# kokkos/kokkos-kernels

Hardware: AMD Instinct MI355X
Metric: SpMV GFLOP/s (CSR, 27-pt 3-D FE Laplacian, fp64) (higher is better)
Workload: dtype f64

## Files before the change

kokkos-kernels_amd/csrc/kk_spmv.hip:

```cpp
#include "kk_common.h"
#include "kk_scan.h"
#include <new>
#include <cstring>
#include <climits>

#include "kk_spmv_plan.h"

namespace kk {

template <class OffT, class AT, class YT, int LPR>
__global__ __launch_bounds__(kBlock) void spmv_vector_kernel(int64_t nrows, const OffT* __restrict__ row_map,
                                                             const int32_t* __restrict__ entries,
                                                             const AT* __restrict__ values, const YT* __restrict__ x,
                                                             YT* __restrict__ y, YT alpha, YT beta, int remap) {
  constexpr int RPB = kBlock / LPR;
  const int64_t wg  = remap ? xcd_remap(blockIdx.x, gridDim.x) : (int64_t)blockIdx.x;
  const int64_t row = wg * RPB + threadIdx.x / LPR;
  const int lane    = threadIdx.x % LPR;
  YT sum            = YT(0);
  if (row < nrows) {
    const OffT s = row_map[row], e = row_map[row + 1];
    for (OffT j = s + lane; j < e; j += LPR) sum += (YT)values[j] * x[entries[j]];
  }
  sum = group_sum(sum, LPR);
// ... 440 lines not shown
  const int mode = tinfo[b] & 3;
  if (mode == kTilePattern) { if (threadIdx.x == 0) tinfo[b] = mode | (int32_t)((unsigned)b << 2); return; }
  if (mode != kTileCodes && mode != kTileStaged) return;
  const int64_t d = idx[b];
  const kk_u32x4* src = reinterpret_cast<const kk_u32x4*>(full + b * TILE);
  kk_u32x4* dst       = reinterpret_cast<kk_u32x4*>(compact + d * TILE);
  for (int i = threadIdx.x; i < TILE / 8; i += kBlock) dst[i] = src[i];
  if (threadIdx.x == 0) tinfo[b] = mode | (int32_t)((unsigned)d << 2);
}

template <class AT, int STEPS, bool FULL, bool NT = false>
__device__ __forceinline__ void load_tile_values(const AT* __restrict__ values, int64_t ts, int64_t te, int t, AT (&v0)[STEPS],
                                                 AT (&v1)[STEPS]) {
  using AV = typename vec2<AT>::type;
  constexpr int SPAN = kBlock * 2;
  KK_UNROLL
  for (int k = 0; k < STEPS; ++k) {
    const int64_t idx = ts + (int64_t)k * SPAN + t * 2;
    if (FULL || idx + 1 < te) {
      const AV* vp = reinterpret_cast<const AV*>(values + idx);
      const AV vv  = NT ? KK_NT_LOAD(vp) : *vp;
      v0[k] = vv[0]; v1[k] = vv[1];
    } else if (idx < te) {
      v0[k] = values[idx]; v1[k] = AT(0);
    } else {
      v0[k] = v1[k] = AT(0);
    }
  }
}

template <int STEPS, bool NT = false>
__device__ __forceinline__ void load_tile_codes(const uint16_t* __restrict__ wtile, int t, unsigned (&w)[STEPS]) {
  constexpr int NPT = 2 * STEPS;
  const unsigned* cw = reinterpret_cast<const unsigned*>(wtile + t * NPT);
  if (STEPS % 4 == 0) {
    KK_UNROLL
    for (int k = 0; k < STEPS; k += 4) {
      const kk_u32x4* qp = reinterpret_cast<const kk_u32x4*>(cw + k);
      const kk_u32x4 q   = NT ? KK_NT_LOAD(qp) : *qp;
      w[k] = q[0]; w[k + 1] = q[1]; w[k + 2] = q[2]; w[k + 3] = q[3];
    }
  } else {
    KK_UNROLL
    for (int k = 0; k < STEPS; k += 2) {
      const kk_u32x2* qp = reinterpret_cast<const kk_u32x2*>(cw + k);
      const kk_u32x2 q   = NT ? KK_NT_LOAD(qp) : *qp;
      w[k] = q[0]; w[k + 1] = q[1];
    }
  }
}

#ifdef KK_EMU
#define KK_USE_AFTER_ISSUE(v)
#else
#define KK_USE_AFTER_ISSUE(v) asm volatile("" : "+v"(v))
#endif

template <class AT, int STEPS, bool FULL>
__device__ __forceinline__ void load_tile_win(const AT* __restrict__ values, const uint16_t* __restrict__ wtile,
                                              const int32_t* __restrict__ wmeta, int64_t b, int64_t ts, int64_t te, int t,
                                              AT (&v0)[STEPS], AT (&v1)[STEPS], int (&c0)[STEPS], int (&c1)[STEPS]) {
  constexpr int SPAN = kBlock * 2;
  unsigned w[STEPS];
  load_tile_codes<STEPS>(wtile, t, w);
  const int meta = wmeta[b * kWinMeta + (t & (kWinMeta - 1))];
  load_tile_values<AT, STEPS, FULL>(values, ts, te, t, v0, v1);
  KK_UNROLL
  for (int k = 0; k < STEPS; ++k) KK_USE_AFTER_ISSUE(w[k]);
  KK_UNROLL
  for (int k = 0; k < STEPS; ++k) {
    const int64_t idx = ts + (int64_t)k * SPAN + t * 2;
    const unsigned lo = w[k] & 0xffffu, hi = w[k] >> 16;
    const int b0 = __shfl(meta, (int)(lo >> kWinBits), 64), b1 = __shfl(meta, (int)(hi >> kWinBits), 64);
    c0[k] = b0 + (int)(lo & ((1u << kWinBits) - 1));
    c1[k] = b1 + (int)(hi & ((1u << kWinBits) - 1));
    if (!FULL) {
      if (idx >= te) c0[k] = c1[k] = -1;
      else if (idx + 1 >= te) c1[k] = c0[k];
    }
  }
}

template <class AT, int STEPS> struct WinTile { AT v0[STEPS], v1[STEPS]; unsigned w[STEPS]; int meta, prec0; };

template <class AT, int STEPS, bool FULL, bool NT, bool PAT>
__device__ __forceinline__ void win_issue(const AT* __restrict__ values, const uint16_t* __restrict__ wtile,
                                          const int32_t* __restrict__ wmeta, const int32_t* __restrict__ pmeta, int64_t b,
                                          int64_t ts, int64_t te, int t, WinTile<AT, STEPS>& W) {
  W.meta  = wmeta[b * kWinMeta + (t & 63)];
  W.prec0 = 0;
  if (PAT) W.prec0 = pmeta[b * kPatW + (t < kPatW ? t : kPatW - 1)];
  load_tile_values<AT, STEPS, FULL, NT>(values, ts, te, t, W.v0, W.v1);
  if (!PAT) load_tile_codes<STEPS, NT>(wtile, t, W.w);
}

template <class AT, class YT, int STEPS, bool PAT>
__device__ __forceinline__ void win_stage(WinTile<AT, STEPS>& W, const YT* __restrict__ x, int64_t ncols, YT* prod, int64_t b, int t,
                                          const int32_t* __restrict__ pmeta) {
  constexpr int SPAN = kBlock * 2, NPT = 2 * STEPS, TILE = kBlock * NPT;
  constexpr int CAPC = (TILE < kWinChunks * 64 ? TILE : kWinChunks * 64) / 64;
  constexpr int CPW  = (CAPC + kBlock / 64 - 1) / (kBlock / 64);
  constexpr int GRP  = STEPS < 4 ? STEPS : 4;
  const AT (&v0)[STEPS] = W.v0;
  const AT (&v1)[STEPS] = W.v1;
  const unsigned (&w)[STEPS] = W.w;
  const int lane = t & 63, wave = t >> 6;
  const int meta = W.meta;
  const int32_t* pm = PAT ? pmeta + b * kPatW : nullptr;
  const int nseg    = PAT ? pm[0] : 0;
  YT xv[CPW];
  bool used[CPW];
  KK_UNROLL
  for (int i = 0; i < CPW; ++i) {
    const int c   = wave + i * (kBlock / 64);
    const int col = c < CAPC ? __shfl(meta, 2 * kWinCount + c, 64) : -1;
    used[i]       = col >= 0;
    int64_t xi    = (int64_t)(used[i] ? col : 0) + lane;
    xi            = xi < ncols ? xi : ncols - 1;
    xv[i]         = x[xi];
  }
  KK_UNROLL
  for (int i = 0; i < CPW; ++i) {
    const int c = wave + i * (kBlock / 64);
    if (used[i]) prod[c * 64 + lane] = xv[i];
  }
  int* sseg = reinterpret_cast<int*>(prod + TILE) - kPatW;
  const short* stab = reinterpret_cast<const short*>(sseg + kPatTab);
  if (PAT && t < kPatW) sseg[t] = W.prec0;
  __syncthreads();
  YT x0[STEPS], x1[STEPS];
  if (PAT) {
    if (nseg == 1) {
      const int jadd = pm[kPatRec + 1];
      const unsigned L = (unsigned)pm[kPatRec + 2];
      const float rcp  = __int_as_float(pm[kPatRec + 3]);
      KK_UNROLL
      for (int k = 0; k < STEPS; ++k) {
        KK_UNROLL
        for (int h = 0; h < 2; ++h) {
          const unsigned j   = (unsigned)(k * SPAN + t * 2 + h + jadd);
          const unsigned row = (unsigned)(((float)j + 0.5f) * rcp);
          const int slot     = (int)stab[(int)(j - KK_UMUL24(row, L))] + (int)row;
          if (h == 0) x0[k] = prod[slot]; else x1[k] = prod[slot];
        }
      }
    } else if (nseg <= 4) {
      const int sb1 = pm[1], sb2 = pm[2], sb3 = pm[3];
      const int ja0 = pm[kPatRec + 1], ja1 = pm[kPatRec + 5], ja2 = pm[kPatRec + 9], ja3 = pm[kPatRec + 13];
      const int sl0 = pm[kPatRec + 2], sl1 = pm[kPatRec + 6], sl2 = pm[kPatRec + 10], sl3 = pm[kPatRec + 14];
      const int sm0 = pm[kPatRec + 3], sm1 = pm[kPatRec + 7], sm2 = pm[kPatRec + 11], sm3 = pm[kPatRec + 15];
      KK_UNROLL
      for (int k0 = 0; k0 < STEPS; k0 += GRP) {
        int ti[2 * GRP], rw[2 * GRP], sl[2 * GRP];
        KK_UNROLL
        for (int q = 0; q < 2 * GRP; ++q) {
          const int li  = (k0 + q / 2) * SPAN + t * 2 + (q & 1);
          const bool c1 = li >= sb1, c2 = li >= sb2, c3 = li >= sb3;
          const int ja  = c3 ? ja3 : c2 ? ja2 : c1 ? ja1 : ja0;
          const int sl_ = c3 ? sl3 : c2 ? sl2 : c1 ? sl1 : sl0;
          const int sm  = c3 ? sm3 : c2 ? sm2 : c1 ? sm1 : sm0;
          const int tb  = c3 ? 3 * kPatLen : c2 ? 2 * kPatLen : c1 ? kPatLen : 0;
          const unsigned j   = (unsigned)(li + ja);
          const unsigned row = (unsigned)(((float)j + 0.5f) * __int_as_float(sm));
          ti[q] = tb + (int)(j - KK_UMUL24(row, (unsigned)sl_));
          rw[q] = (int)row;
        }
        KK_UNROLL
        for (int q = 0; q < 2 * GRP; ++q) sl[q] = (int)stab[ti[q]] + rw[q];
        KK_UNROLL
        for (int q = 0; q < 2 * GRP; ++q) {
          if ((q & 1) == 0) x0[k0 + q / 2] = prod[sl[q]]; else x1[k0 + q / 2] = prod[sl[q]];
        }
      }
    } else {
      const int sb1 = pm[1], sb2 = pm[2], sb3 = pm[3], sb4 = pm[4], sb5 = pm[5], sb6 = pm[6], sb7 = pm[7];
      KK_UNROLL
// ... 79 lines not shown
      vb[k] = quad_pick<0xFA, AT>(v0[k], v1[k], odd);
    }
    KK_UNROLL
    for (int k = 0; k < STEPS; ++k) {
      const int li = k * SPAN + t * 2 - j;
      prod[li]     = (YT)va[k] * xa[k];
      prod[li + 4] = (YT)vb[k] * xb[k];
    }
    return;
  }
  YT x0[STEPS], x1[STEPS];
  KK_UNROLL
  for (int k = 0; k < STEPS; ++k) {
    x0[k] = (FULL || c0[k] >= 0) ? x[FULL ? c0[k] : (c0[k] >= 0 ? c0[k] : 0)] : YT(0);
    x1[k] = (FULL || c1[k] >= 0) ? x[FULL ? c1[k] : (c1[k] >= 0 ? c1[k] : 0)] : YT(0);
  }
  KK_UNROLL
  for (int k = 0; k < STEPS; ++k) {
    const int li = k * SPAN + t * 2;
    prod[li]     = (YT)v0[k] * x0[k];
    prod[li + 1] = (YT)v1[k] * x1[k];
  }
}

template <class YT> __device__ __forceinline__ YT strided_lds_sum(const YT* prod, int i0, int i1, int lane, int G) {
  YT s0 = YT(0), s1 = YT(0), s2 = YT(0), s3 = YT(0);
  int i = i0 + lane;
  const int G2 = 2 * G, G3 = 3 * G, G4 = 4 * G;
  for (; i + G3 < i1; i += G4) {
    const YT a = prod[i], b = prod[i + G], c = prod[i + G2], d = prod[i + G3];
    s0 += a; s1 += b; s2 += c; s3 += d;
  }
  for (; i < i1; i += G) s0 += prod[i];
  return (s0 + s1) + (s2 + s3);
}

template <class OffT, class AT, class YT, int NPT, int MODE>
__global__ __launch_bounds__(kBlock) void spmv_stream3_kernel(int64_t nnz, const OffT* __restrict__ row_map,
                                                              const int32_t* __restrict__ entries,
                                                              const AT* __restrict__ values, const YT* __restrict__ x,
                                                              YT* __restrict__ y, YT alpha, YT beta,
                                                              const int32_t* __restrict__ blk_info,
                                                              YT* __restrict__ carry_head, YT* __restrict__ carry_tail,
                                                              int remap, const int32_t* __restrict__ list,
                                                              const int32_t* __restrict__ tinfo,
                                                              const uint16_t* __restrict__ wcode,
                                                              const int32_t* __restrict__ wmeta, int64_t ncols,
                                                              const int32_t* __restrict__ pmeta KK_ABL_PARAM) {
  constexpr int TILE  = kBlock * NPT;
  constexpr int STEPS = NPT / 2;
  __shared__ YT prod[TILE];
  constexpr bool NT = false;
  const int t       = threadIdx.x;
  const int64_t pos = xcd_order(blockIdx.x, gridDim.x, remap);
  const int64_t b   = list ? (int64_t)list[pos] : pos;
  const int64_t s = b * TILE;
  const bool full = (s + TILE <= nnz);
  const int64_t e = full ? s + TILE : nnz;

  const int32_t info0 = blk_info[b], info1 = blk_info[b + 1];
  const uint16_t* wtile = nullptr;
  if (MODE == kTileCodes || MODE == kTileStaged) wtile = wcode + (int64_t)((unsigned)tinfo[b] >> 2) * TILE;

  AT v0[STEPS], v1[STEPS];
  int c0[STEPS], c1[STEPS];
  WinTile<AT, STEPS> W;
  if (MODE == kTilePattern) {
    win_issue<AT, STEPS, true, NT, true>(values, wtile, wmeta, pmeta, b, s, e, t, W);
  } else if (MODE == kTileStaged) {
    if (full) win_issue<AT, STEPS, true, NT, false>(values, wtile, wmeta, pmeta, b, s, e, t, W);
    else      win_issue<AT, STEPS, false, NT, false>(values, wtile, wmeta, pmeta, b, s, e, t, W);
  } else if (MODE == kTileCodes) {
    if (full) load_tile_win<AT, STEPS, true>(values, wtile, wmeta, b, s, e, t, v0, v1, c0, c1);
    else      load_tile_win<AT, STEPS, false>(values, wtile, wmeta, b, s, e, t, v0, v1, c0, c1);
  } else {
    if (full) load_tile<AT, STEPS, NT, true>(values, entries, s, e, t, v0, v1, c0, c1);
    else      load_tile<AT, STEPS, NT, false>(values, entries, s, e, t, v0, v1, c0, c1);
  }

  const int64_t ra    = info0 & 0x7fffffff;
  const int64_t rb    = info1 & 0x7fffffff;
  const int has_head  = (info0 >> 31) & 1;
  const int64_t nv    = (rb - ra) + has_head;
  int G = 1;
  while (G < kWave && nv * (G * 2) <= kBlock) G *= 2;
  const int lane = t & (G - 1), grp = t / G, ngrp = kBlock / G;
  bool valid = grp < nv;
  int64_t r  = ra + grp - has_head;
  int64_t rc = r > 0 ? r : 0;
  rc         = rc < rb ? rc : rb - 1;
  OffT rs_raw = OffT(0), re_raw = OffT(0);
  if (!KK_ABL(16)) { rs_raw = row_map[rc]; re_raw = row_map[rc + 1]; }
  YT yold = YT(0);
  if (beta != YT(0)) yold = y[rc];

  if (MODE >= kTileStaged) {
    win_stage<AT, YT, STEPS, MODE == kTilePattern>(W, x, ncols, prod, b, t, pmeta);
  } else {
    if (full) stage_products<AT, YT, STEPS, true, true>(x, prod, t, v0, v1, c0, c1);
    else      stage_products<AT, YT, STEPS, false, false>(x, prod, t, v0, v1, c0, c1);
  }
  if (!KK_ABL(32)) __syncthreads();

  int64_t rs = 0, re = 0;
  if (valid) {
    if (KK_ABL(16)) { rs = s + (int64_t)grp * 27; re = rs + 27; }
    else { rs = (int64_t)rs_raw; re = (int64_t)re_raw; }
  }
  for (int64_t base = 0; base < nv; base += ngrp) {
    if (base > 0) {
      valid = (base + grp) < nv;
      r     = ra + base + grp - has_head;
      if (valid) { rs = (int64_t)row_map[r]; re = (int64_t)row_map[r + 1]; }
    }
    const bool is_head  = r < ra;
    const bool complete = !is_head && re <= e;
    const int i0 = (int)((rs > s ? rs : s) - s), i1 = (int)((re < e ? re : e) - s);
    YT sum = valid ? (KK_ABL(8) ? prod[i0 < TILE ? i0 : 0] : strided_lds_sum<YT>(prod, i0, i1, lane, G)) : YT(0);
    sum = group_sum(sum, G);
    if (valid && lane == 0) {
      if (is_head) carry_head[b] = sum;
      else if (!complete) carry_tail[b] = sum;
      else if (!KK_ABL(4) && !(KK_ABL(64) && (b & 7))) {
        sum *= alpha;
// ... 464 lines not shown
  else if (k == "mv5_min_fill_pct") { if (value < 0 || value > 100) return bad("a percentage"); t.mv5_min_fill_pct = value; }
  else if (k == "mv5_max_other_pct") { if (value < 0 || value > 100) return bad("a percentage"); t.mv5_max_other_pct = value; }
  else if (k == "stream_variant") { if (value != 1 && value != 6) return bad("1 or 6"); t.stream_variant = value; }
  else if (k == "mv_remap") { if (!valid_order_knob(value)) return bad("0, 1 or a power of two"); t.mv_remap = value; }
  else if (k == "mv_order") { if (value < 0 || value > 2) return bad("in 0..2"); t.mv_order = value; }
  else if (k == "mv_strip_min_kb") { if (value < 0) return bad("non-negative"); t.mv_strip_min_kb = value; }
  else if (k == "mv_strip_l2_kb") { if (value < 1) return bad("positive"); t.mv_strip_l2_kb = value; }
  else if (k == "mv_nt") { if (value != 0 && value != 1) return bad("0 or 1"); t.mv_nt = value; }
  else if (k == "mv_glds") { if (value != 0 && value != 1) return bad("0 or 1"); t.mv_glds = value; }
  else if (k == "mv_long_T") { if (value < 0) return bad("non-negative"); t.mv_long_T = value; }
  else if (k == "mv4_min_nvec") { if (value < 1 || value > 1024) return bad("in 1..1024"); t.mv4_min_nvec = value; }
  else if (k == "mv4_2d") { if (value != 0 && value != 1) return bad("0 or 1"); t.mv4_2d = value; }
  else if (k == "mv4_xcol") { if (value != 0 && value != 1) return bad("0 or 1"); t.mv4_xcol = value; }
  else if (k == "mv4_wg_per_cu") { if (value < 1 || value > 64) return bad("in 1..64"); t.mv4_wg_per_cu = value; }
  else if (k == "march") { if (value != 0 && value != 1) return bad("0 or 1"); t.march = value; }
  else if (k == "march_planes") { if (value < 1 || value > 4096) return bad("in 1..4096"); t.march_planes = value; }
  else if (k == "window_codes") { if (value < 0 || value > 2) return bad("in 0..2"); t.window_codes = value; }
  else if (k == "window_codes_min_knnz") { if (value < 0) return bad("non-negative"); t.window_codes_min_knnz = value; }
  else if (k == "window_codes_min_pct") { if (value < 0 || value > 100) return bad("a percentage"); t.window_codes_min_pct = value; }
  else if (k == "pattern_codes") { if (value < 0 || value > 2) return bad("in 0..2"); t.pattern_codes = value; }
  else if (k == "pattern_direct") { if (value != 0 && value != 1) return bad("0 or 1"); t.pattern_direct = value; }
  else if (k == "pattern_codes_min_knnz") { if (value < 0) return bad("non-negative"); t.pattern_codes_min_knnz = value; }
  else if (k == "colslab") { if (value < 0 || value > 4) return bad("in 0..4"); t.colslab = value; }
  else if (k == "colslab_min_pct") { if (value < 0 || value > 100) return bad("in 0..100"); t.colslab_min_pct = value; }
  else if (k == "colslab_min_knnz") { if (value < 0) return bad("non-negative"); t.colslab_min_knnz = value; }
  else if (k == "colslab_shift") { if (value != 0 && (value < 2 || value > 30)) return bad("0 or in 2..30"); t.colslab_shift = value; }
  else if (k == "colslab_rate_pct") { if (value < 1 || value > 1000) return bad("in 1..1000"); t.colslab_rate_pct = value; }
  else if (k == "values_tracking") { if (value < 0 || value > 2) return bad("in 0..2"); t.values_tracking = value; }
  else if (k == "check_entries") { if (value != 0 && value != 1) return bad("0 or 1"); t.check_entries = value; }
  else if (k == "defer_rank1") { if (value != 0 && value != 1) return bad("0 or 1"); t.defer_rank1 = value; }
  else if (k == "colslab_const") { if (value != 0 && value != 1) return bad("0 or 1"); t.colslab_const = value; }
  else if (k == "transient_min_knnz") { if (value < 0) return bad("non-negative"); t.transient_min_knnz = value; }
  else if (k == "explicit_transpose") { if (value < 0 || value > 2) return bad("in 0..2"); t.explicit_transpose = value; }
  else if (k == "explicit_transpose_min_knnz") { if (value < 0) return bad("non-negative"); t.explicit_transpose_min_knnz = value; }
#ifdef KK_ABLATE
  else if (k == "ablate") t.ablate = value;
  else if (k == "lds_pad_kb") t.lds_pad_kb = value;
#endif
  else return fail(KKAMD_ERR_INVALID_ARG, "unknown tuning key '%s'", key);
  return KKAMD_OK;
}

template <class OffT>
static int analyse(kkamd_spmv_plan* p, const kkamd_crs_t* A, hipStream_t st) {
  KK_LAUNCH((spmv_plan_kernel<OffT>), (unsigned)ceil_div(p->nblocks + 1, kBlock), kBlock, 0, st, A->num_rows,
            (const OffT*)A->d_row_map, p->nblocks, (int64_t)p->tile, p->d_blk_row);
  KK_LAUNCH_CHECK();
  return KKAMD_OK;
}

static void free_analysis(kkamd_spmv_plan* p) {
  void** bufs[] = {(void**)&p->d_blk_row, &p->d_carry, (void**)&p->d_tinfo, (void**)&p->d_wcode, (void**)&p->d_wbase, (void**)&p->d_pmeta};
  for (void** b : bufs) if (*b) { (void)hipFree(*b); *b = nullptr; }
  for (int m = 0; m < 4; ++m) { if (p->d_list[m]) { (void)hipFree(p->d_list[m]); p->d_list[m] = nullptr; } p->n_mode[m] = 0; }
  p->pat_tiles = p->code_tiles = p->staged_tiles = p->plain_tiles = 0; p->pat_direct = false;
  p->tile = 0; p->nblocks = 0; p->plan_bytes = 0;
}

static int build_codes(kkamd_spmv_plan* p, const kkamd_crs_t* A, hipStream_t st, int npt, bool may_retile, int* redo_npt) {
  *redo_npt = 0;
  const size_t nb = (size_t)p->nblocks;
  DevBuf full, counts, flag, tinfo_b, wbase_b;
  auto give_up = [&]() {
    (void)hipGetLastError();
    if (p->d_pmeta) { (void)hipFree(p->d_pmeta); p->d_pmeta = nullptr; }
    if (p->d_wcode) { (void)hipFree(p->d_wcode); p->d_wcode = nullptr; }
    for (int m = 0; m < 4; ++m) { if (p->d_list[m]) { (void)hipFree(p->d_list[m]); p->d_list[m] = nullptr; } p->n_mode[m] = 0; }
    p->d_tinfo = nullptr; p->d_wbase = nullptr;
    p->pat_tiles = p->code_tiles = p->staged_tiles = 0; p->plain_tiles = p->nblocks;
    p->win_failed = true;
    return KKAMD_OK;
  };
  if (full.alloc(sizeof(uint16_t) * nb * (size_t)p->tile) != hipSuccess || counts.alloc(12 * sizeof(int)) != hipSuccess ||
      flag.alloc(sizeof(int32_t) * (nb + 1)) != hipSuccess || tinfo_b.alloc(sizeof(int32_t) * nb) != hipSuccess ||
      wbase_b.alloc(sizeof(int32_t) * nb * kWinMeta) != hipSuccess)
    return give_up();
  int32_t* tinfo = tinfo_b.as<int32_t>();
  int32_t* wbase = wbase_b.as<int32_t>();
  uint16_t* d_full = full.as<uint16_t>();
  int* d_counts    = counts.as<int>();
  int32_t* d_flag  = flag.as<int32_t>();
  KK_HIP(hipMemsetAsync(counts.p, 0, 12 * sizeof(int), st));
  const int allow_stage = p->tune.window_codes != 2;
  const int32_t* ent = (const int32_t*)p->entries;
  auto make_lists = [&](const int64_t* known, size_t* list_bytes) -> int {
    for (int m = 0; m < 4; ++m) {
      if (known && known[m] == 0) { p->n_mode[m] = 0; continue; }
      if (known && known[m] == (int64_t)nb) { p->n_mode[m] = (int64_t)nb; continue; }
      KK_LAUNCH(mode_flag_kernel, (unsigned)ceil_div((int64_t)nb + 1, kBlock), kBlock, 0, st, (int64_t)nb, (const int32_t*)tinfo, d_flag, m);
      if (hipGetLastError() != hipSuccess) return -1;
      int rc2 = exclusive_scan_inplace<int32_t>(d_flag, (int64_t)nb + 1, st);
      if (rc2) { give_up(); return rc2; }
      int32_t cnt = 0;
      if (known) cnt = (int32_t)known[m];
      else {
        KK_HIP(hipMemcpyAsync(&cnt, d_flag + nb, sizeof(int32_t), hipMemcpyDeviceToHost, st));
        KK_HIP(hipStreamSynchronize(st));
      }
      p->n_mode[m] = cnt;
      if (cnt > 0 && (size_t)cnt < nb) {
        if (hipMalloc((void**)&p->d_list[m], sizeof(int32_t) * (size_t)cnt) != hipSuccess) return -1;
        *list_bytes += sizeof(int32_t) * (size_t)cnt;
        int32_t* d_list_m = p->d_list[m];
        KK_LAUNCH(mode_scatter_kernel, (unsigned)ceil_div((int64_t)nb, kBlock), kBlock, 0, st, (int64_t)nb, (const int32_t*)tinfo, (const int32_t*)d_flag, d_list_m, m);
        if (hipGetLastError() != hipSuccess) return -1;
      }
    }
    return 0;
  };
  const bool pat_wanted = p->tune.pattern_codes && (npt == 16 || npt == 8) &&
                          (p->tune.pattern_codes >= 2 || A->nnz >= (int64_t)p->tune.pattern_codes_min_knnz * 1000);
  if (pat_wanted && allow_stage && p->tune.pattern_direct && hipMalloc((void**)&p->d_pmeta, sizeof(int32_t) * nb * kPatW) == hipSuccess) {
    const bool o64 = A->offset_type == KKAMD_I64;
    int* d_cnt = d_counts + 8;
#define KK_PAT_DIRECT(OT, N)                                                                                                 \
  KK_LAUNCH((pat_direct_kernel<OT, N>), (unsigned)nb, kBlock, 0, st, A->nnz, (const OT*)A->d_row_map, ent,                   \
            (const int32_t*)p->d_blk_row, wbase, tinfo, p->d_pmeta)
    if (npt == 16) { if (o64) { KK_PAT_DIRECT(int64_t, 16); } else { KK_PAT_DIRECT(int32_t, 16); } }
    else           { if (o64) { KK_PAT_DIRECT(int64_t, 8); } else { KK_PAT_DIRECT(int32_t, 8); } }
#undef KK_PAT_DIRECT
    if (hipGetLastError() != hipSuccess) return give_up();
    KK_LAUNCH(tile_mode_hist_kernel, (unsigned)ceil_div((int64_t)nb, kBlock), kBlock, 0, st, (int64_t)nb, (const int32_t*)tinfo, d_cnt);
    if (hipGetLastError() != hipSuccess) return give_up();
    int hd[4] = {0, 0, 0, 0};
    KK_HIP(hipMemcpyAsync(hd, d_cnt, 4 * sizeof(int), hipMemcpyDeviceToHost, st));
    KK_HIP(hipStreamSynchronize(st));
    const int64_t left = (int64_t)nb - hd[kTilePattern], allowed = (int64_t)nb / 100 > 1 ? (int64_t)nb / 100 : 1;
    if (hd[kTilePattern] > 0 && left <= allowed) {
      if (hipMalloc((void**)&p->d_wcode, sizeof(uint16_t) * (size_t)p->tile) != hipSuccess) return give_up();
      const int64_t known[4] = {left, 0, 0, (int64_t)hd[kTilePattern]};
      size_t list_bytes = 0;
      int rc2 = make_lists(known, &list_bytes);
      if (rc2) return rc2 == -1 ? give_up() : rc2;
      KK_HIP(hipStreamSynchronize(st));
      p->d_tinfo = (int32_t*)tinfo_b.release(); p->d_wbase = (int32_t*)wbase_b.release();
      p->plain_tiles = left; p->pat_tiles = hd[kTilePattern]; p->code_tiles = 0; p->staged_tiles = hd[kTilePattern]; p->pat_direct = true;
      p->plan_bytes += list_bytes + sizeof(int32_t) * nb * (1 + kWinMeta) + sizeof(uint16_t) * (size_t)p->tile + sizeof(int32_t) * nb * kPatW;
      return KKAMD_OK;
    }
    KK_HIP(hipFree(p->d_pmeta)); p->d_pmeta = nullptr;
  } else {
    (void)hipGetLastError();
    if (p->d_pmeta) { (void)hipFree(p->d_pmeta); p->d_pmeta = nullptr; }
  }
  if (npt == 16)     { KK_LAUNCH((win_build_kernel<16>), (unsigned)nb, kBlock, 0, st, A->nnz, ent, d_full, wbase, tinfo, allow_stage); }
  else if (npt == 8) { KK_LAUNCH((win_build_kernel<8>), (unsigned)nb, kBlock, 0, st, A->nnz, ent, d_full, wbase, tinfo, allow_stage); }
  else               { KK_LAUNCH((win_build_kernel<4>), (unsigned)nb, kBlock, 0, st, A->nnz, ent, d_full, wbase, tinfo, allow_stage); }
  if (hipGetLastError() != hipSuccess) return give_up();
  KK_LAUNCH(tile_mode_hist_kernel, (unsigned)ceil_div((int64_t)nb, kBlock), kBlock, 0, st, (int64_t)nb, (const int32_t*)tinfo, d_counts);
  if (hipGetLastError() != hipSuccess) return give_up();
  int h[8] = {0};
  KK_HIP(hipMemcpyAsync(h, counts.p, 4 * sizeof(int), hipMemcpyDeviceToHost, st));
  KK_HIP(hipStreamSynchronize(st));
// ... 276 lines not shown
  if (t.mv_long_T != old.mv_long_T && plan->mv_long_known) {
    if (plan->used) KK_HIP(hipStreamSynchronize(plan->last_stream));
    if (plan->d_mv_long) { KK_HIP(hipFree(plan->d_mv_long)); plan->d_mv_long = nullptr; }
    plan->mv_long_known = false; plan->n_mv_long = 0; plan->mv_long_T = 0; plan->mv_long_nnz = 0;
  }
  return KKAMD_OK;
}

int kkamd_spmv_plan_values_changed(kkamd_spmv_plan_t* plan) {
  if (!plan) return kk::fail(KKAMD_ERR_INVALID_ARG, "kkamd_spmv_plan_values_changed: null plan");
  plan->t_stale = true;
  kk::cs_mark_stale(plan->cs);
  return KKAMD_OK;
}

int kkamd_spmv_plan_query(const kkamd_spmv_plan_t* plan, const char* key, int64_t* value) {
  if (!plan || !key || !value) return kk::fail(KKAMD_ERR_INVALID_ARG, "kkamd_spmv_plan_query: null argument");
  const std::string k(key);
  if (k.rfind("transpose_plan_", 0) == 0) {
    if (!plan->t_plan) { *value = 0; return KKAMD_OK; }
    return kkamd_spmv_plan_query(plan->t_plan, k.c_str() + 15, value);
  }
  if (k == "tile") *value = plan->tile;
  else if (k == "tiles") *value = plan->nblocks;
  else if (k == "window_codes") *value = plan->d_tinfo ? 1 : 0;
  else if (k == "window_staged_x") *value = (plan->d_tinfo && plan->staged_tiles > 0) ? 1 : 0;
  else if (k == "plain_tiles") *value = plan->d_tinfo ? plan->plain_tiles : plan->nblocks;
  else if (k == "code_tiles") *value = plan->code_tiles;
  else if (k == "staged_tiles") *value = plan->d_tinfo ? plan->staged_tiles : 0;
  else if (k == "pattern_tiles") *value = plan->d_pmeta ? plan->pat_tiles : 0;
  else if (k == "plan_bytes") *value = (int64_t)plan->plan_bytes;
  else if (k == "transpose_bytes") {
    const int64_t ob = plan->offset_type == KKAMD_I64 ? 8 : 4, vb = plan->value_type == KKAMD_F64 ? 8 : 4;
    *value = plan->t_ready ? plan->nnz * (4 + ob + vb) + (plan->num_cols + 1) * ob + 16 * kk::values_fp_tiles(plan->nnz) + (plan->d_t_shadow ? plan->nnz * vb : 0) : 0;
  }
  else if (k == "transpose_cached") *value = plan->t_ready ? 1 : 0;
  else if (k == "mv_tiles") *value = kk::mv_plan_query(plan->mv, 0);
  else if (k == "mv_staged_tiles") *value = kk::mv_plan_query(plan->mv, 1);
  else if (k == "mv_long_rows") *value = plan->n_mv_long;
  else if (k == "mv_order") *value = plan->mv ? kk::mv_plan_query(plan->mv, 2) : (plan->d_mv2_order ? 2 : 0);
  else if (k == "mv_period") *value = plan->mv_period;
  else if (k == "mv_plan_bytes") *value = kk::mv_plan_query(plan->mv, 3) + kk::mv4_plan_query(plan->mv4, 3) + kk::mv5_plan_query(plan->mv5, 3) + kk::mv6_plan_query(plan->mv6, 2);
  else if (k == "mv4_workgroups") *value = kk::mv4_plan_query(plan->mv4, 0);
  else if (k == "mv4_other_rows") *value = kk::mv4_plan_query(plan->mv4, 1);
  else if (k == "mv4_stencil") *value = kk::mv4_plan_query(plan->mv4, 2);
  else if (k == "mv4_near_stride") *value = kk::mv4_plan_query(plan->mv4, 4);
  else if (k == "mv6_chunks") *value = kk::mv6_plan_query(plan->mv6, 0);
  else if (k == "mv6_empty_rows") *value = kk::mv6_plan_query(plan->mv6, 1);
  else if (k == "mv_long_nnz") *value = plan->mv_long_nnz;
  else if (k == "mv5_tiles") *value = kk::mv5_plan_query(plan->mv5, 0);
  else if (k == "mv5_other_rows") *value = kk::mv5_plan_query(plan->mv5, 1);
  else if (k == "mv5_blocks") *value = kk::mv5_plan_query(plan->mv5, 2);
  else if (k == "mv5_fill_permille") *value = kk::mv5_plan_query(plan->mv5, 4);
  else if (k == "pattern_direct") *value = plan->pat_direct ? 1 : 0;
  else if (k == "colslab") *value = plan->cs ? 1 : 0;
  else if (k == "colslab_tried") *value = plan->cs_tried ? 1 : 0;
  else if (k == "colslab_slabs") *value = kk::cs_plan_query(plan->cs, 0);
  else if (k == "colslab_shift") *value = kk::cs_plan_query(plan->cs, 1);
  else if (k == "colslab_bytes") *value = kk::cs_plan_query(plan->cs, 2);
  else if (k == "colslab_deterministic") *value = kk::cs_plan_query(plan->cs, 3);
  else if (k == "colslab_lines_permille") *value = (int64_t)(plan->cs_ratio * 1000.0 + 0.5);
  else if (k == "colslab_crs_us") *value = (int64_t)(plan->cs_crs_us + 0.5);
  else if (k == "colslab_us") *value = (int64_t)(plan->cs_us + 0.5);
  else if (k == "march_workgroups") *value = plan->tune.march ? kk::mv4_plan_query(plan->mv4, 5) : 0;
  else return kk::fail(KKAMD_ERR_INVALID_ARG, "kkamd_spmv_plan_query: unknown key '%s'", key);
  return KKAMD_OK;
}

int kkamd_spmv_plan_export(const kkamd_spmv_plan_t* plan, const char* what, void* h_out, int64_t count) {
  if (!plan || !what || !h_out) return kk::fail(KKAMD_ERR_INVALID_ARG, "kkamd_spmv_plan_export: null argument");
  const std::string k(what);
  const void* src = nullptr; int64_t have = 0; size_t esz = 4;
  if (k == "tile_first_row") { src = plan->d_blk_row; have = plan->d_blk_row ? plan->nblocks + 1 : 0; }
  else if (k == "tile_mode") { src = plan->d_tinfo; have = plan->d_tinfo ? plan->nblocks : 0; }
  else return kk::fail(KKAMD_ERR_INVALID_ARG, "kkamd_spmv_plan_export: unknown array '%s'", what);
  if (count > have) return kk::fail(KKAMD_ERR_INVALID_ARG, "kkamd_spmv_plan_export: '%s' has %lld entries, %lld asked for", what, (long long)have, (long long)count);
  if (count > 0) KK_HIP(hipMemcpy(h_out, src, esz * (size_t)count, hipMemcpyDeviceToHost));
  return KKAMD_OK;
}

int kkamd_release_scratch(void) { const int rc = kk::release_transient(); const int rc2 = kk::release_bitmap_pool(); return rc ? rc : rc2; }

int kkamd_spmv(kkamd_spmv_plan_t* plan, const kkamd_crs_t* A, char mode, double alpha, const void* d_x, double beta,
               void* d_y, int vector_type, kkamd_stream_t stream) {
  int rc = kk::check_crs(A);
  if (rc) return rc;
  bool trans = false;
  if ((rc = kk::parse_mode(mode, &trans))) return rc;
  if ((rc = kk::check_plan(plan, A))) return rc;
  if (vector_type != KKAMD_F32 && vector_type != KKAMD_F64)
    return kk::fail(KKAMD_ERR_UNSUPPORTED, "kkamd_spmv: unsupported vector_type %d", vector_type);
  if (A->value_type == KKAMD_F64 && vector_type != KKAMD_F64)
    return kk::fail(KKAMD_ERR_UNSUPPORTED, "kkamd_spmv: unsupported (value,vector) type pair (%d,%d)", A->value_type, vector_type);
  hipStream_t st     = kk::to_hip(stream);
  const int64_t ylen = trans ? A->num_cols : A->num_rows;
  const int64_t xlen = trans ? A->num_rows : A->num_cols;
  if (ylen > 0 && !d_y) return kk::fail(KKAMD_ERR_INVALID_ARG, "kkamd_spmv: null y");
  if (alpha == 0.0 || A->num_rows == 0 || A->num_cols == 0 || A->nnz == 0) {
    if (vector_type == KKAMD_F64) return kk::launch_scale<double>((double*)d_y, ylen, 1, 1, 1, beta, st);
    return kk::launch_scale<float>((float*)d_y, ylen, 1, 1, 1, (float)beta, st);
  }
  if (xlen > 0 && !d_x) return kk::fail(KKAMD_ERR_INVALID_ARG, "kkamd_spmv: null x");
  if ((rc = kk::bind_stream(plan, st))) return rc;
  if ((rc = kk::check_entries_content(plan, A, st))) return rc;
  kk::TraceRange range(A->value_type == KKAMD_F64 ? "KokkosSparse::spmv[TPL_KKAMD,double]" : "KokkosSparse::spmv[TPL_KKAMD,float]");
  KK_DISPATCH_TYPES(kk::spmv_typed, plan, A, trans, alpha, d_x, beta, d_y, st);
// ... 4 lines not shown
```

kokkos-kernels_amd/csrc/kk_spmv_plan.h:

```cpp
#pragma once
#include "kk_common.h"
#include <string>
#include <utility>
#include <vector>

#ifdef KK_ABLATE
#define KK_ABL_PARAM , int ablate
#define KK_ABL_ARG(p) , (p)->tune.ablate
#define KK_ABL(bit) ((ablate & (bit)) != 0)
#define KK_LDS_PAD(p) ((size_t)(p)->tune.lds_pad_kb * 1024)
#else
#define KK_ABL_PARAM
#define KK_ABL_ARG(p)
#define KK_ABL(bit) false
#define KK_LDS_PAD(p) ((size_t)0)
#endif

namespace kk {

struct SpmvTuning {
  int kernel         = 0;
  int lanes_per_row  = 0;
  int nnz_per_thread = 0;
  int xcd_remap      = 16;
// ... 26 lines not shown
  int window_codes_min_pct = 25;
  int pattern_codes = 1;
  int pattern_direct = 1;
  int pattern_codes_min_knnz = 10000;
  int colslab = 3;
  int colslab_min_pct = 85;
  int colslab_min_knnz = 20000;
  int colslab_shift = 0;
  int colslab_rate_pct = 61;
  int defer_rank1 = 0;
  int check_entries = 0;
  int colslab_const = 0;
  int values_tracking = 0;
#ifdef KK_ABLATE
  int ablate         = 0;
  int lds_pad_kb     = 0;
#endif
};
extern SpmvTuning g_spmv_default;

inline bool valid_order_knob(int v) { return v == 0 || v == 1 || (v >= 2 && v <= (1 << 20) && (v & (v - 1)) == 0); }

}

constexpr int kTilePlain = 0, kTileCodes = 1, kTileStaged = 2, kTilePattern = 3;

struct kkamd_mv_plan;
struct kkamd_mv4_plan;
struct kkamd_cs_plan;
struct kkamd_mv5_plan;
struct kkamd_mv6_plan;

struct kkamd_spmv_plan {
  std::vector<std::pair<std::string, int>> set_log;
  int64_t num_rows = 0, num_cols = 0, nnz = 0;
  const void* row_map = nullptr;
  int offset_type = 0, value_type = 1, algorithm = 0;
  kk::SpmvTuning tune;
  int tile = 0;
  int64_t nblocks = 0;
  int num_cus = 256;
  int32_t* d_blk_row = nullptr;
  void* d_carry = nullptr;
  void* d_xpack = nullptr;
  size_t xpack_bytes = 0;
  void* d_ypack = nullptr;
  size_t ypack_bytes = 0;
  const void* entries = nullptr;
  int32_t* d_tinfo = nullptr;
  uint16_t* d_wcode = nullptr;
  int32_t* d_wbase = nullptr;
  int32_t* d_pmeta = nullptr;
  int32_t* d_list[4] = {nullptr, nullptr, nullptr, nullptr};
  int64_t n_mode[4]  = {0, 0, 0, 0};
  int64_t code_tiles = 0;
  int64_t staged_tiles = 0;
  int64_t pat_tiles = 0;
  bool pat_direct = false;
  int64_t plain_tiles = 0;
  size_t plan_bytes = 0;
  void* d_t_rm = nullptr; int32_t* d_t_ent = nullptr; void* d_t_perm = nullptr; void* d_t_val = nullptr; unsigned long long* d_t_fp = nullptr;
  kkamd_spmv_plan* t_plan = nullptr;
  void* d_t_shadow = nullptr;
  bool t_ready = false, t_failed = false, t_fp_valid = false, t_shadow_valid = false, t_shadow_failed = false, t_stale = true;
  bool rank1_deferred = false;
  bool win_failed = false;
  kkamd_mv_plan* mv = nullptr;
  bool mv_failed = false;
  kkamd_mv4_plan* mv4 = nullptr;
  bool mv4_tried = false;
  kkamd_mv5_plan* mv5 = nullptr;
  bool mv5_tried = false;
  kkamd_mv6_plan* mv6 = nullptr;
  bool mv6_tried = false;
  int32_t* d_mv2_order = nullptr;
  int32_t* d_mv_long = nullptr; int64_t n_mv_long = 0, mv_long_T = 0, mv_long_nnz = 0; bool mv_long_known = false;
  kkamd_cs_plan* cs = nullptr;
  bool cs_tried = false;
  double cs_crs_us = 0.0, cs_us = 0.0;
  double cs_ratio = 0.0;
  int mv2_rb = 0;
  bool mv2_tried = false, mv_period_known = false;
  int64_t mv_period = 0;
  hipStream_t last_stream = nullptr;
  bool used = false;
  unsigned long long entries_hash = 0; bool entries_hash_known = false;
};

namespace kk {
int  bind_stream(kkamd_spmv_plan* p, hipStream_t st);
int  check_plan(const kkamd_spmv_plan* p, const kkamd_crs_t* A);
int  check_entries_content(kkamd_spmv_plan* p, const kkamd_crs_t* A, hipStream_t st);
void mv_plan_destroy(kkamd_mv_plan* mv);
int64_t mv_plan_query(const kkamd_mv_plan* mv, int what);
void mv4_plan_destroy(kkamd_mv4_plan* p);
int64_t mv4_plan_query(const kkamd_mv4_plan* p, int what);
void mv5_plan_destroy(kkamd_mv5_plan* p);
int64_t mv5_plan_query(const kkamd_mv5_plan* p, int what);
int  mv5_plan_build(kkamd_spmv_plan* plan, const kkamd_crs_t* A, hipStream_t st);
int  mv5_spmv(const kkamd_spmv_plan* plan, const kkamd_crs_t* A, const double* X, int64_t xs0, int64_t xs1, double* Y, int64_t ys0, int64_t ys1,
              int64_t nvec, double alpha, double beta, hipStream_t st);
void mv6_plan_destroy(kkamd_mv6_plan* p);
int64_t mv6_plan_query(const kkamd_mv6_plan* p, int what);
int  mv6_plan_build(kkamd_spmv_plan* plan, const kkamd_crs_t* A, hipStream_t st);
int  mv6_spmv(kkamd_spmv_plan* plan, const kkamd_crs_t* A, const double* X, int64_t ldx, double* Y, int64_t ys0, int64_t ys1,
              int64_t nvec, double alpha, double beta, hipStream_t st);
// ... 59 lines not shown
```

Measured before the change: 1162.

## Prefetch x window chunks at tile issue for pattern tiles, skip identity tile lists

Result: faster. 1261 (median of 6 runs) (+8.5%).

```diff
diff --git a/kokkos-kernels_amd/csrc/kk_spmv.hip b/kokkos-kernels_amd/csrc/kk_spmv.hip
--- a/kokkos-kernels_amd/csrc/kk_spmv.hip
+++ b/kokkos-kernels_amd/csrc/kk_spmv.hip
@@ -516,8 +516,10 @@
 
 #ifdef KK_EMU
 #define KK_USE_AFTER_ISSUE(v)
+#define KK_USE_SCALAR_AFTER_ISSUE(v)
 #else
 #define KK_USE_AFTER_ISSUE(v) asm volatile("" : "+v"(v))
+#define KK_USE_SCALAR_AFTER_ISSUE(v) asm volatile("" : "+s"(v))
 #endif
 
 template <class AT, int STEPS, bool FULL>
@@ -545,25 +547,50 @@
   }
 }
 
-template <class AT, int STEPS> struct WinTile { AT v0[STEPS], v1[STEPS]; unsigned w[STEPS]; int meta, prec0; };
-
-template <class AT, int STEPS, bool FULL, bool NT, bool PAT>
+template <int STEPS> struct WinGeom {
+  static constexpr int TILE = kBlock * 2 * STEPS;
+  static constexpr int CAPC = (TILE < kWinChunks * 64 ? TILE : kWinChunks * 64) / 64;
+  static constexpr int CPW  = (CAPC + kBlock / 64 - 1) / (kBlock / 64);
+};
+template <class AT, class YT, int STEPS> struct WinTile {
+  AT v0[STEPS], v1[STEPS];
+  unsigned w[STEPS];
+  int meta, prec0, ccol[WinGeom<STEPS>::CPW];
+  YT xv[WinGeom<STEPS>::CPW];
+};
+
+template <class AT, class YT, int STEPS, bool FULL, bool NT, bool PAT>
 __device__ __forceinline__ void win_issue(const AT* __restrict__ values, const uint16_t* __restrict__ wtile,
-                                          const int32_t* __restrict__ wmeta, const int32_t* __restrict__ pmeta, int64_t b,
-                                          int64_t ts, int64_t te, int t, WinTile<AT, STEPS>& W) {
-  W.meta  = wmeta[b * kWinMeta + (t & 63)];
+                                          const int32_t* __restrict__ wmeta, const int32_t* __restrict__ pmeta,
+                                          const YT* __restrict__ x, int64_t ncols, int64_t b, int64_t ts, int64_t te, int t,
+                                          WinTile<AT, YT, STEPS>& W) {
+  constexpr int CPW = WinGeom<STEPS>::CPW;
+  W.meta  = 0;
   W.prec0 = 0;
-  if (PAT) W.prec0 = pmeta[b * kPatW + (t < kPatW ? t : kPatW - 1)];
+  if (PAT) {
+    static_assert(!PAT || CPW * (kBlock / 64) == WinGeom<STEPS>::CAPC, "every wave stages CPW chunks of the window");
+    const int32_t* cm = wmeta + b * kWinMeta + 2 * kWinCount + KK_UNIFORM(t >> 6) * CPW;
+    KK_UNROLL
+    for (int i = 0; i < CPW; ++i) W.ccol[i] = cm[i];
+    KK_UNROLL
+    for (int i = 0; i < CPW; ++i) {
+      int64_t xi = (int64_t)(W.ccol[i] >= 0 ? W.ccol[i] : 0) + (t & 63);
+      xi         = xi < ncols ? xi : ncols - 1;
+      W.xv[i]    = x[xi];
+    }
+    W.prec0 = pmeta[b * kPatW + (t < kPatW ? t : kPatW - 1)];
+  } else {
+    W.meta = wmeta[b * kWinMeta + (t & 63)];
+  }
   load_tile_values<AT, STEPS, FULL, NT>(values, ts, te, t, W.v0, W.v1);
   if (!PAT) load_tile_codes<STEPS, NT>(wtile, t, W.w);
 }
 
 template <class AT, class YT, int STEPS, bool PAT>
-__device__ __forceinline__ void win_stage(WinTile<AT, STEPS>& W, const YT* __restrict__ x, int64_t ncols, YT* prod, int64_t b, int t,
+__device__ __forceinline__ void win_stage(WinTile<AT, YT, STEPS>& W, const YT* __restrict__ x, int64_t ncols, YT* prod, int64_t b, int t,
                                           const int32_t* __restrict__ pmeta) {
   constexpr int SPAN = kBlock * 2, NPT = 2 * STEPS, TILE = kBlock * NPT;
-  constexpr int CAPC = (TILE < kWinChunks * 64 ? TILE : kWinChunks * 64) / 64;
-  constexpr int CPW  = (CAPC + kBlock / 64 - 1) / (kBlock / 64);
+  constexpr int CAPC = WinGeom<STEPS>::CAPC, CPW = WinGeom<STEPS>::CPW;
   constexpr int GRP  = STEPS < 4 ? STEPS : 4;
   const AT (&v0)[STEPS] = W.v0;
   const AT (&v1)[STEPS] = W.v1;
@@ -576,16 +603,17 @@
   bool used[CPW];
   KK_UNROLL
   for (int i = 0; i < CPW; ++i) {
-    const int c   = wave + i * (kBlock / 64);
-    const int col = c < CAPC ? __shfl(meta, 2 * kWinCount + c, 64) : -1;
+    const int c   = PAT ? wave * CPW + i : wave + i * (kBlock / 64);
+    const int col = PAT ? W.ccol[i] : c < CAPC ? __shfl(meta, 2 * kWinCount + c, 64) : -1;
     used[i]       = col >= 0;
+    if (PAT) { xv[i] = W.xv[i]; continue; }
     int64_t xi    = (int64_t)(used[i] ? col : 0) + lane;
     xi            = xi < ncols ? xi : ncols - 1;
     xv[i]         = x[xi];
   }
   KK_UNROLL
   for (int i = 0; i < CPW; ++i) {
-    const int c = wave + i * (kBlock / 64);
+    const int c = PAT ? wave * CPW + i : wave + i * (kBlock / 64);
     if (used[i]) prod[c * 64 + lane] = xv[i];
   }
   int* sseg = reinterpret_cast<int*>(prod + TILE) - kPatW;
@@ -771,6 +799,9 @@
   __shared__ YT prod[TILE];
   constexpr bool NT = false;
   const int t       = threadIdx.x;
+  if (MODE == kTilePattern) {
+    KK_USE_SCALAR_AFTER_ISSUE(alpha); KK_USE_SCALAR_AFTER_ISSUE(beta); KK_USE_SCALAR_AFTER_ISSUE(ncols);
+  }
   const int64_t pos = xcd_order(blockIdx.x, gridDim.x, remap);
   const int64_t b   = list ? (int64_t)list[pos] : pos;
   const int64_t s = b * TILE;
@@ -783,12 +814,12 @@
 
   AT v0[STEPS], v1[STEPS];
   int c0[STEPS], c1[STEPS];
-  WinTile<AT, STEPS> W;
+  WinTile<AT, YT, STEPS> W;
   if (MODE == kTilePattern) {
-    win_issue<AT, STEPS, true, NT, true>(values, wtile, wmeta, pmeta, b, s, e, t, W);
+    win_issue<AT, YT, STEPS, true, NT, true>(values, wtile, wmeta, pmeta, x, ncols, b, s, e, t, W);
   } else if (MODE == kTileStaged) {
-    if (full) win_issue<AT, STEPS, true, NT, false>(values, wtile, wmeta, pmeta, b, s, e, t, W);
-    else      win_issue<AT, STEPS, false, NT, false>(values, wtile, wmeta, pmeta, b, s, e, t, W);
+    if (full) win_issue<AT, YT, STEPS, true, NT, false>(values, wtile, wmeta, pmeta, x, ncols, b, s, e, t, W);
+    else      win_issue<AT, YT, STEPS, false, NT, false>(values, wtile, wmeta, pmeta, x, ncols, b, s, e, t, W);
   } else if (MODE == kTileCodes) {
     if (full) load_tile_win<AT, STEPS, true>(values, wtile, wmeta, b, s, e, t, v0, v1, c0, c1);
     else      load_tile_win<AT, STEPS, false>(values, wtile, wmeta, b, s, e, t, v0, v1, c0, c1);
@@ -1359,7 +1390,7 @@
 static void free_analysis(kkamd_spmv_plan* p) {
   void** bufs[] = {(void**)&p->d_blk_row, &p->d_carry, (void**)&p->d_tinfo, (void**)&p->d_wcode, (void**)&p->d_wbase, (void**)&p->d_pmeta};
   for (void** b : bufs) if (*b) { (void)hipFree(*b); *b = nullptr; }
-  for (int m = 0; m < 4; ++m) { if (p->d_list[m]) { (void)hipFree(p->d_list[m]); p->d_list[m] = nullptr; } p->n_mode[m] = 0; }
+  for (int m = 0; m < 4; ++m) { if (p->d_list[m]) { (void)hipFree(p->d_list[m]); p->d_list[m] = nullptr; } p->n_mode[m] = 0; p->list_identity[m] = false; }
   p->pat_tiles = p->code_tiles = p->staged_tiles = p->plain_tiles = 0; p->pat_direct = false;
   p->tile = 0; p->nblocks = 0; p->plan_bytes = 0;
 }
@@ -1372,7 +1403,7 @@
     (void)hipGetLastError();
     if (p->d_pmeta) { (void)hipFree(p->d_pmeta); p->d_pmeta = nullptr; }
     if (p->d_wcode) { (void)hipFree(p->d_wcode); p->d_wcode = nullptr; }
-    for (int m = 0; m < 4; ++m) { if (p->d_list[m]) { (void)hipFree(p->d_list[m]); p->d_list[m] = nullptr; } p->n_mode[m] = 0; }
+    for (int m = 0; m < 4; ++m) { if (p->d_list[m]) { (void)hipFree(p->d_list[m]); p->d_list[m] = nullptr; } p->n_mode[m] = 0; p->list_identity[m] = false; }
     p->d_tinfo = nullptr; p->d_wbase = nullptr;
     p->pat_tiles = p->code_tiles = p->staged_tiles = 0; p->plain_tiles = p->nblocks;
     p->win_failed = true;
@@ -1392,8 +1423,9 @@
   const int32_t* ent = (const int32_t*)p->entries;
   auto make_lists = [&](const int64_t* known, size_t* list_bytes) -> int {
     for (int m = 0; m < 4; ++m) {
+      p->list_identity[m] = false;
       if (known && known[m] == 0) { p->n_mode[m] = 0; continue; }
-      if (known && known[m] == (int64_t)nb) { p->n_mode[m] = (int64_t)nb; continue; }
+      if (known && known[m] == (int64_t)nb) { p->n_mode[m] = (int64_t)nb; p->list_identity[m] = true; continue; }
       KK_LAUNCH(mode_flag_kernel, (unsigned)ceil_div((int64_t)nb + 1, kBlock), kBlock, 0, st, (int64_t)nb, (const int32_t*)tinfo, d_flag, m);
       if (hipGetLastError() != hipSuccess) return -1;
       int rc2 = exclusive_scan_inplace<int32_t>(d_flag, (int64_t)nb + 1, st);
@@ -1405,7 +1437,15 @@
         KK_HIP(hipStreamSynchronize(st));
       }
       p->n_mode[m] = cnt;
-      if (cnt > 0 && (size_t)cnt < nb) {
+      if (cnt > 0) {
+        int32_t lead = cnt;
+        if ((size_t)cnt < nb) {
+          KK_HIP(hipMemcpyAsync(&lead, d_flag + cnt, sizeof(int32_t), hipMemcpyDeviceToHost, st));
+          KK_HIP(hipStreamSynchronize(st));
+        }
+        p->list_identity[m] = lead == cnt;
+      }
+      if (cnt > 0 && !p->list_identity[m]) {
         if (hipMalloc((void**)&p->d_list[m], sizeof(int32_t) * (size_t)cnt) != hipSuccess) return -1;
         *list_bytes += sizeof(int32_t) * (size_t)cnt;
         int32_t* d_list_m = p->d_list[m];
@@ -1788,6 +1828,7 @@
   else if (k == "mv5_other_rows") *value = kk::mv5_plan_query(plan->mv5, 1);
   else if (k == "mv5_blocks") *value = kk::mv5_plan_query(plan->mv5, 2);
   else if (k == "mv5_fill_permille") *value = kk::mv5_plan_query(plan->mv5, 4);
+  else if (k == "pattern_list_identity") *value = (plan->d_tinfo && plan->d_pmeta && plan->n_mode[kTilePattern] > 0 && plan->list_identity[kTilePattern]) ? 1 : 0;
   else if (k == "pattern_direct") *value = plan->pat_direct ? 1 : 0;
   else if (k == "colslab") *value = plan->cs ? 1 : 0;
   else if (k == "colslab_tried") *value = plan->cs_tried ? 1 : 0;
diff --git a/kokkos-kernels_amd/csrc/kk_spmv_plan.h b/kokkos-kernels_amd/csrc/kk_spmv_plan.h
--- a/kokkos-kernels_amd/csrc/kk_spmv_plan.h
+++ b/kokkos-kernels_amd/csrc/kk_spmv_plan.h
@@ -102,6 +102,7 @@
   int32_t* d_wbase = nullptr;
   int32_t* d_pmeta = nullptr;
   int32_t* d_list[4] = {nullptr, nullptr, nullptr, nullptr};
+  bool list_identity[4] = {false, false, false, false};
   int64_t n_mode[4]  = {0, 0, 0, 0};
   int64_t code_tiles = 0;
   int64_t staged_tiles = 0;
```
